# inverted-ai/torchdrivesim

Measured on AMD Instinct MI355X. Metric: agent-steps/sec (whole node) at B=1024xA=64, 256x256 BEV, higher is better.
Workload: dtype f32

## Files before the change

include/tdship.h:

```cpp
#ifndef TDSHIP_H
#define TDSHIP_H

#include <stddef.h>
#include <stdint.h>

#ifdef __cplusplus
extern "C" {
#endif

#define TDS_ABI_VERSION 1

#define TDS_OK 0
#define TDS_EINVAL (-1)
#define TDS_EHIP (-2)
#define TDS_ENOMEM (-3)
#define TDS_ELIMIT (-4)

int tds_version(void);
int tds_last_error(char *buf, size_t n);


int tds_bicycle_step_f32(const float *state, const float *action, const float *lr, float *out, int64_t n,
                         float dt, float max_acc, float max_steer, int left_handed, int no_reversing, void *stream);
int tds_bicycle_step_bwd_f32(const float *state, const float *action, const float *lr, const float *grad_out,
// ... 299 lines not shown
int tds_time_to_collision_f32(const float *boxes, const float *sc, const float *speed, const uint8_t *present, const uint8_t *visible,
                              float *ttc, int32_t *index, int64_t B, int64_t A, int64_t E, int K, float horizon, float margin, void *stream);

int tds_time_to_collision_bwd_f32(const float *boxes, const float *sc, const float *speed, const int32_t *index, const float *g_ttc,
                                  float *g_boxes, float *g_sc, float *g_speed, int64_t B, int64_t A, int64_t E, int K, float margin, void *stream);

#define TDS_RASTER_DBG_NO_STATIC 1
#define TDS_RASTER_DBG_NO_ACTORS 2
#define TDS_RASTER_DBG_NO_STORE 4
#define TDS_RASTER_DBG_NO_EDGES 8
#define TDS_RASTER_DBG_NO_SCAN 16
#define TDS_RASTER_DBG_NO_BINNED 32
#define TDS_RASTER_DBG_NO_BITS 64
#define TDS_RASTER_DBG_STATS 128
#define TDS_RASTER_DBG_NO_EDGE_WALK 256
#define TDS_RASTER_DBG_NO_SETUP 512
#define TDS_RASTER_DBG_NO_PROJECT 1024
#define TDS_RASTER_DBG_MINWG3 2048
#define TDS_RASTER_DBG_XCD_CLOCKS 4096
#define TDS_RASTER_DBG_NO_SPLIT 8192
#define TDS_RASTER_DBG_SPLIT 16384
#define TDS_RASTER_DBG_NO_SHORT_PATH 32768
#define TDS_RASTER_DBG_GRID8 65536
#define TDS_RASTER_DBG_GRID4 131072
#define TDS_RASTER_DBG_WHOLE_4WAVES 262144
#define TDS_RASTER_DBG_NO_8WAVES 524288
#define TDS_RASTER_DBG_WIDEST_STRIPS 1048576
#define TDS_RASTER_DBG_NO_EXTRA_STRIP 2097152
#define TDS_RASTER_DBG_PROLOGUE_TWICE 4194304
#define TDS_RASTER_DBG_DROP_SMALL 8388608
#define TDS_RASTER_DBG_SMALL_FREE_SLOPES 16777216
#define TDS_RASTER_DBG_SMALL_NO_MIDDLE_ROW 33554432
#define TDS_RASTER_DBG_HELPER 67108864
#ifndef TDS_RASTER_SMALL_ROWS
#define TDS_RASTER_SMALL_ROWS 7
#endif

#ifdef TDS_TESTING
int tds_raster_set_strip_width(int tw);
int tds_raster_set_bits_waves(int n);
int tds_raster_set_list_lds(int lds_kb);
int tds_raster_set_list_waves(int waves);
int tds_raster_set_debug(int flags);
int tds_raster_set_helper_min_items(int items_per_workgroup);
int tds_raster_get_helper_stats(unsigned long long *out1);
int tds_raster_get_stats(unsigned long long *out16);
int tds_raster_get_prep_stats(unsigned long long *out2);
int tds_raster_get_small_stats(unsigned long long *out16);
typedef struct {
    int form, tw, strips, twp, nwv, nb, minwg, emit, four_per_cu, persist, tws, lw;
    int64_t lds, lds_s, grid, caps, off_counts, off_lists, off_lists3;
} tds_raster_plan_t;
int tds_raster_plan(int64_t n_img, int res, int out_mode, int n_keys, int keys_listed, int actors, int extra, int want_slices, int64_t workspace_bytes,
                    int cus, int force_tw, int bits_waves, int list_waves, int list_lds_kb, int debug, tds_raster_plan_t *out);
int tds_raster_plan_small_lane(int64_t n_img, int res, int out_mode, int n_keys, int keys_listed, int actors, int extra, int want_slices,
                               int64_t workspace_bytes, int cus, int force_tw, int bits_waves, int list_waves, int list_lds_kb, int debug,
                               int small_faces, int *small_lane);
int tds_testing_set_near_lists(int enabled);
int tds_stop_lines_bwd_set_row_lanes(int lanes);
#endif

#ifdef __cplusplus
}
#endif
#endif
```

torchdrivesim_amd/_native.py:

```python
import contextlib
import ctypes
import enum
import functools
import os
import re
import subprocess

import torch

_HERE = os.path.dirname(os.path.abspath(__file__))
LIB_PATH = os.path.join(_HERE, 'lib', 'libtdship.so')
TESTING_LIB_PATH = os.path.join(_HERE, 'lib', 'libtdship_testing.so')
CSRC = os.path.join(_HERE, 'csrc')

METRIC_IOU, METRIC_DISCS = 0, 1
OUT_F32, OUT_U8 = 0, 1
OUT_MASK_U8, OUT_MASK_BITS = 2, 3
RASTER_NO_TRIM = 1
RASTER_REWRITE_ALL = 2
RASTER_HAS_CAMERA_PREP = 4
RASTER_NO_SMALL_FACES = 8
RASTER_HAS_HELPER_STREAM = 16


class RasterDebug(enum.IntFlag):
    NO_STATIC = 1
    NO_ACTORS = 2
    NO_STORE = 4
    NO_EDGES = 8
    NO_SCAN = 16
    NO_BINNED = 32
    NO_BITS = 64
    STATS = 128
    NO_EDGE_WALK = 256
    NO_SETUP = 512
    NO_PROJECT = 1024
    MINWG3 = 2048
    XCD_CLOCKS = 4096
    NO_SPLIT = 8192
    SPLIT = 16384
    NO_SHORT_PATH = 32768
    GRID8 = 65536
    GRID4 = 131072
    WHOLE_4WAVES = 262144
    NO_8WAVES = 524288
    WIDEST_STRIPS = 1048576
    NO_EXTRA_STRIP = 2097152
    PROLOGUE_TWICE = 4194304
    DROP_SMALL = 8388608
    SMALL_FREE_SLOPES = 16777216
    SMALL_NO_MIDDLE_ROW = 33554432
    HELPER = 67108864

_lib = None


class RasterAux(ctypes.Structure):
    _fields_ = [('index_slices', ctypes.c_void_p), ('index_slices_bytes', ctypes.c_int64), ('keys', ctypes.c_uint32 * 16),
                ('n_keys', ctypes.c_int32), ('index_bits', ctypes.c_int32), ('flags', ctypes.c_int32), ('coverage_maintained', ctypes.c_int32),
                ('coverage', ctypes.c_void_p), ('coverage_bytes', ctypes.c_int64)]


class RasterAuxPrep(RasterAux):
    _fields_ = [('camera_prep', ctypes.c_void_p), ('camera_prep_bytes', ctypes.c_int64)]


class RasterAuxHelper(RasterAuxPrep):
    _fields_ = [('helper_stream', ctypes.c_void_p), ('helper_workgroups', ctypes.c_int64)]


_ABI = '''
tds_version()
tds_last_error(host* buf, size_t n)
tds_bicycle_step_f32(f32* state, f32* action, f32* lr, f32* out, int64 n, float dt, float max_acc, float max_steer, int left_handed, int no_reversing, stream stream)
tds_bicycle_step_bwd_f32(f32* state, f32* action, f32* lr, f32* grad_out, f32* grad_state, f32* grad_action, f32* grad_lr, int64 n, float dt, float max_acc, float max_steer,
    int left_handed, int no_reversing, stream stream)
tds_simple_step_f32(f32* state, f32* action, f32* out, int64 n, float dt, host* norm, int oriented, stream stream)
tds_simple_step_bwd_f32(f32* state, f32* action, f32* grad_out, f32* grad_state, f32* grad_action, int64 n, float dt, host* norm, int oriented, stream stream)
tds_unicycle_step_f32(f32* state, f32* action, f32* out, int64 n, float dt, float max_acc, float max_yaw_rate, stream stream)
tds_unicycle_step_bwd_f32(f32* state, f32* action, f32* grad_out, f32* grad_state, f32* grad_action, int64 n, float dt, float max_acc, float max_yaw_rate, stream stream)
tds_collision_f32(f32* boxes, f32* sc, u8* present, f32* out, i64* overlap, i32* partner, int64 B, int64 A, int64 N, int metric, stream stream)
tds_collision_bwd_f32(f32* boxes, f32* sc, u8* present, f32* grad_out, f32* grad_boxes, f32* grad_sc, int64 B, int64 A, int64 N, int metric, stream stream)
tds_overlap_count_f32(f32* boxes, f32* sc, u8* present, f64* out, int64 B, int64 A, stream stream)
tds_pairwise_overlap_f32(f32* box1, f32* sc1, f32* box2, f32* sc2, f32* out, int64 n, int metric, stream stream)
tds_pairwise_discs_f32(f32* box1, f32* sc1, f32* box2, f32* sc2, f32* out, int64 n, int num_discs, stream stream)
# ... 97 lines not shown
tds_range_scan_multi_f32(handle set, i32* scene_map, f32* boxes, f32* sc, u8* present, f32* ray_sc, f32* agent_range, f32* road_range, i32* hit, int64 B, int64 A, int64 E,
    int R, float max_range, float gap_tolerance, stream stream)
tds_range_scan_bwd_f32(handle map, f32* boxes, f32* sc, u8* present, f32* ray_sc, f32* road_range, f32* g_agent, f32* g_road, f32* g_boxes, f32* g_sc, f32* g_ray_sc,
    i32* choice, f32* road_edge, int64 B, int64 A, int64 E, int R, float max_range, float gap_tolerance, stream stream)
tds_range_scan_bwd_multi_f32(handle set, i32* scene_map, f32* boxes, f32* sc, u8* present, f32* ray_sc, f32* road_range, f32* g_agent, f32* g_road, f32* g_boxes, f32* g_sc,
    f32* g_ray_sc, i32* choice, f32* road_edge, int64 B, int64 A, int64 E, int R, float max_range, float gap_tolerance, stream stream)
tds_neighbors_f32(f32* boxes, f32* sc, f32* speed, u8* present, u8* visible, f32* features, i32* index, int64 B, int64 A, int64 E, int K, float max_distance, stream stream)
tds_neighbors_bwd_f32(f32* boxes, f32* sc, f32* speed, i32* index, f32* g_features, f32* g_boxes, f32* g_sc, f32* g_speed, int64 B, int64 A, int64 E, int K, stream stream)
tds_lights_step(f64* duration, i32* next_phase, i32* n_phases, u8* colour, i32* phase, f64* remaining, i64* state, f32* time_to_change, u8* mask, int64 B, int64 M, int64 P,
    int64 N, host* dt, int advance, stream stream)
tds_lights_reset(i32* n_phases, f64* duration, i32* phase, f64* remaining, u8* mask, i64* scene_ids, int64 B, int64 M, int64 P, uint64 seed, stream stream)
tds_stop_lines_f32(f32* agent_xy, f32* agent_sc, u8* agent_present, f32* lines, f32* line_sc, u8* mask, i64* state, f32* time_to_change, f32* features, i32* index,
    i32* slot_state, int64 B, int64 A, int64 N, int K, float max_distance, int ahead_only, float min_cos, stream stream)
tds_stop_lines_bwd_f32(f32* agent_xy, f32* agent_sc, f32* lines, f32* line_sc, i32* index, f32* g_features, f32* g_xy, f32* g_sc, int64 B, int64 A, int64 N, int K,
    stream stream)
tds_lane_observations_multi(handle set, i32* scene_map, f32* agent_xy, f32* agent_sc, u8* present, f32* features, f32* points, i32* n_valid, i32* index, int64 B, int64 A,
    int K, int P, float spacing, float max_distance, stream stream)
tds_lane_observations_bwd_multi(handle set, i32* scene_map, f32* agent_xy, f32* agent_sc, i32* index, f32* g_features, f32* g_points, f32* g_xy, f32* g_sc, int64 B, int64 A,
    int K, int P, float spacing, stream stream)
tds_time_to_collision_f32(f32* boxes, f32* sc, f32* speed, u8* present, u8* visible, f32* ttc, i32* index, int64 B, int64 A, int64 E, int K, float horizon,
    float margin, stream stream)
tds_time_to_collision_bwd_f32(f32* boxes, f32* sc, f32* speed, i32* index, f32* g_ttc, f32* g_boxes, f32* g_sc, f32* g_speed, int64 B, int64 A, int64 E, int K,
    float margin, stream stream)
'''

_TESTING_ABI = '''
tds_raster_set_strip_width(int tw)
tds_raster_set_bits_waves(int n)
tds_raster_set_list_lds(int lds_kb)
tds_raster_set_list_waves(int waves)
tds_raster_set_debug(int flags)
tds_raster_set_helper_min_items(int items_per_workgroup)
tds_raster_get_helper_stats(host* out1)
tds_raster_get_stats(host* out16)
tds_raster_get_prep_stats(host* out2)
tds_raster_get_small_stats(host* out16)
tds_raster_plan(int64 n_img, int res, int out_mode, int n_keys, int keys_listed, int actors, int extra, int want_slices, int64 workspace_bytes, int cus, int force_tw,
    int bits_waves, int list_waves, int list_lds_kb, int debug, host* out)
tds_raster_plan_small_lane(int64 n_img, int res, int out_mode, int n_keys, int keys_listed, int actors, int extra, int want_slices, int64 workspace_bytes, int cus,
    int force_tw, int bits_waves, int list_waves, int list_lds_kb, int debug, int small_faces, host* small_lane)
tds_testing_set_near_lists(int enabled)
tds_stop_lines_bwd_set_row_lanes(int lanes)
'''

ELEMENTS = {'f32*': torch.float32, 'f64*': torch.float64, 'u8*': torch.uint8, 'i32*': torch.int32, 'i64*': torch.int64, 'void*': None}
SCALARS = {'int': ctypes.c_int, 'int64': ctypes.c_int64, 'uint64': ctypes.c_uint64, 'float': ctypes.c_float, 'size_t': ctypes.c_size_t}


def _parse(abi):
    decls = {name: [tuple(p.split()) for p in params.split(',') if p.strip()] for name, params in re.findall(r'(\w+)\((.*?)\)', abi, flags=re.S)}
    assert all(k in ELEMENTS or k in SCALARS or k in ('host*', 'handle', 'stream') for d in decls.values() for k, _ in d)
    return decls


DECLARATIONS, TESTING_DECLARATIONS = _parse(_ABI), _parse(_TESTING_ABI)
_SIGNATURES = {name: [SCALARS.get(k, ctypes.c_void_p) for k, _ in d] for name, d in DECLARATIONS.items()}
_TESTING_SIGNATURES = {name: [SCALARS.get(k, ctypes.c_void_p) for k, _ in d] for name, d in TESTING_DECLARATIONS.items()}
_RESTYPES = {'tds_buffer_ptr': ctypes.c_void_p, 'tds_torch_alloc': ctypes.c_void_p, 'tds_torch_free': None}


def build(force=False):
    cmd = ['make', '-C', CSRC, '-j', str(min(8, os.cpu_count() or 1))]
    if force:
        cmd.append('-B')
    subprocess.check_call(cmd, stdout=subprocess.DEVNULL)
    return LIB_PATH
# ... 121 lines not shown
```

torchdrivesim_amd/csrc/raster.hip:

```cpp
#include "tds_common.h"
#include "tds_face_rows.h"
#include "tds_raster_plan.h"
#include "tds_short_slope.h"
#include <algorithm>
#include <atomic>
#include <mutex>
#include <type_traits>

using tds::GridEntry;
using tds::MapView;
using namespace tds_raster;

#ifdef TDS_TESTING
#define TDS_DBG(x) (x)
#else
#define TDS_DBG(x) 0
#endif

namespace {

constexpr int RBLOCK = RWAVES * 64;
constexpr int NO_SWITCH = 0x7fffffff;
constexpr int COORD_LIMIT = 16000;

struct SceneArgs {
    MapView map;
    const MapView *views;
    const int32_t *scene_map;
    const float4 *state;
    const float2 *agent_sc;
    const float2 *tmpl;
    const uint32_t *actor_key;
// ... 659 lines not shown
    MapView m = a.map;
    if (a.views != nullptr) m = a.views[a.scene_map[img / a.Nc]];
    int cx0 = 0, cx1 = -1, cy0 = 0, nrows = 0, rtotal = 0;
    if (m.nx > 0 && !(TDS_DBG(c.debug) & TDS_RASTER_DBG_NO_STATIC)) {
        int cy1;
        scan_window(m, c, cam, X0, TWp, cx0, cx1, cy0, cy1);
        nrows = (cx0 <= cx1 && cy0 <= cy1) ? cy1 - cy0 + 1 : 0;
    }
    if (nrows > 0 && nrows <= PREP_ROWS) {
        ScanQuad q;
        scan_quad(q, c, cam, X0, TWp);
        for (int r = 0; r < nrows; ++r) {
            int rw = SCAN_EMPTY_ROW, rfe = 0, re0 = 0, re1 = 0;
            scan_row(q, m, cx0, cx1, cy0, r, rw, rfe, re0, re1);
            rec.rows[r] = make_int4(rw, rtotal, re0 - rtotal, rfe);
            rtotal += re1 - re0;
        }
    }
    float *f = rec.cam;
    f[0] = cam.cx; f[1] = cam.cy; f[2] = cam.s; f[3] = cam.c;
#pragma unroll
    for (int k = 0; k < 4; ++k) { f[4 + k] = cam.px[k]; f[8 + k] = cam.py[k]; }
    rec.cx0 = cx0; rec.cx1 = cx1; rec.cy0 = cy0; rec.nrows = nrows;
    rec.rtotal = rtotal; rec.flags = nrows > PREP_ROWS ? PREP_COMPUTE : 0; rec.pad0 = 0; rec.pad1 = 0;
}

typedef const __attribute__((address_space(4))) int PrepWords;
__device__ __forceinline__ PrepWords *prep_words(const void *tab, int item) {
    return (PrepWords *)((uintptr_t)tab + (uintptr_t)(unsigned)item * sizeof(PrepRecord));
}

template <typename SA, bool POLY = false>
__device__ __forceinline__ void scan_init(ScanState &st, const SA &a, const CommonArgs &c, const Camera &cam, int64_t img, int lane, int wave, int X0,
                                          int TWw, const PrepRecord *rec = nullptr) {
    st.map = a.map;
    if (a.views != nullptr) st.map = a.views[a.scene_map[img / a.Nc]];
    if constexpr (POLY) st.map.cell_start = st.map.qcell_start;
    const MapView &m = st.map;
    st.phase = (a.N > 0 && !(TDS_DBG(c.debug) & TDS_RASTER_DBG_NO_ACTORS)) ? 0 : 2;
    if constexpr (POLY) {
        st.phase = (a.N > 0 && !(c.debug & TDS_RASTER_DBG_NO_ACTORS)) ? 0 : 2;
    }
    if constexpr (has_extras<SA>::value) { if (st.phase == 2 && a.K > 0) st.phase = 3; }
    st.a0 = 0; st.masked_seen = false;
    st.cx0 = 0; st.cx1 = -1; st.cy0 = 0; st.nrows = 0; st.row = 0; st.chunk = __builtin_amdgcn_readfirstlane(wave); st.prev_rw = SCAN_EMPTY_ROW;
    st.rw = SCAN_EMPTY_ROW; st.rex = st.rbase = st.rfe = 0; st.rtotal = 0;
    st.have = false; st.cur_i = -1; st.dyn = nullptr; st.done = 0;
    st.pu0 = st.pu1 = st.pu2 = make_uint4(0, 0, 0, 0);
    if (m.nx > 0 && !(TDS_DBG(c.debug) & TDS_RASTER_DBG_NO_STATIC)) {
        if (rec != nullptr) {
            PrepWords *w = prep_words(rec, 0);
            st.cx0 = w[12]; st.cx1 = w[13]; st.cy0 = w[14]; st.nrows = w[15]; st.rtotal = w[16];
            st.rex = st.rtotal; st.rbase = -st.rtotal;
            if (lane < st.nrows) {
                const int4 v = rec->rows[lane];
                st.rw = v.x; st.rex = v.y; st.rbase = v.z; st.rfe = v.w;
            }
        } else {
            int cy1;
            scan_window(m, c, cam, X0, TWw, st.cx0, st.cx1, st.cy0, cy1);
            st.nrows = (st.cx0 <= st.cx1 && st.cy0 <= cy1) ? __builtin_amdgcn_readfirstlane(cy1 - st.cy0 + 1) : 0;
            if (st.nrows > 0) scan_load_rows(st, m, c, cam, lane, X0, TWw, 0);
        }
    }
}

template <int NW, bool POLY = false>
__device__ __forceinline__ bool scan_fetch(ScanState &st, const MapView &m, const CommonArgs &c, const Camera &cam, int lane, int X0, int TWw) {
    while (st.row < st.nrows) {
        const int nblk = min(64, st.nrows - st.row);
        const int total = st.rtotal;
        if (st.chunk * 64 < total) {
// ... 44 lines not shown
            const int cand = r + step;
            const int ex = __shfl(st.rex, cand & 63);
            if (cand < nblk && ex <= v) r = cand;
        }
    }
    const int i = __shfl(st.rbase, r) + v;
    return v < st.rtotal ? (i | (r << 25)) : -1;
}

__device__ __forceinline__ void scan_candidate(const ScanState &st, const CommonArgs &c, const Camera &cam, int X0, int TWw, int ci, const uint4 &u0,
                                               const uint4 &u1, bool &acc, uint32_t &key, int (&px)[3], int (&py)[3], unsigned &edges) {
    const int i = ci & 0x1ffffff, r = ci >= 0 ? ci >> 25 : 0;
    const int first_end = __shfl(st.rfe, r);
    const int above = __shfl(st.rw, (r + 63) & 63);
    const int pw = r > 0 ? above : st.prev_rw;
    const int plo = pw & 0xffff, phi = pw >> 16;
    const bool top = st.row + r == 0;
    if (ci >= 0) {
        const unsigned own = u1.w;
        const int bx0 = (int)(own & 0x1fffu), bx1 = (int)((own >> 13) & 0x1fffu);
        const bool first_in_row = !(own & (1u << 26)) || (i < first_end);
        const bool none_above = !(own & (1u << 27)) || top || bx1 < plo || bx0 > phi;
        if (first_in_row && none_above && !(TDS_DBG(c.debug) & TDS_RASTER_DBG_NO_PROJECT)) {
            unsigned ins = 0;
            float sxv[3] = {__uint_as_float(u0.x) + (-cam.cx), __uint_as_float(u0.z) + (-cam.cx), __uint_as_float(u1.x) + (-cam.cx)};
            float syv[3] = {__uint_as_float(u0.y) + (-cam.cy), __uint_as_float(u0.w) + (-cam.cy), __uint_as_float(u1.y) + (-cam.cy)};
            key = u1.z;
            acc = trim_project(cam, c.scale, c.res, X0, TWw, sxv, syv, px, py, ins, c.no_trim);
            edges = edge_mask(own >> 29, ins);
        }
    }
}

template <int NW = RWAVES, typename SA = SceneArgsEx>
__device__ __forceinline__ bool scan_step(ScanState &st, const SA &a, const CommonArgs &c, const Camera &cam, int64_t img, int lane,
                                          int wave, int X0, int TWw, bool &acc, uint32_t &key, int (&px)[3], int (&py)[3], unsigned &edges) {
    const MapView &m = st.map;
    unsigned ins = 0;
    edges = 7u;
    const int res = c.res;
    const int64_t b = img / a.Nc;
    acc = false;
    key = 0;
    if (st.phase == 0) {
        const int slot = lane / 3, f = lane - 3 * slot;
        const int ag = st.a0 + slot * NW + wave;
        if (lane < 63 && ag < a.N) {
            const int64_t ia = b * a.N + ag;
            const bool on = a.mask[img * a.N + ag] != 0;
            st.masked_seen = st.masked_seen || !on;
            if (on) {
                const float view_r = 1.05f * 1.41421356f / c.scale;
                const float4 s = a.state[ia];
                const float2 t0 = a.tmpl[ia * 7];
                float reach = view_r + sqrtf(t0.x * t0.x + t0.y * t0.y);
                reach = reach * 1.01f + 0.01f;
                const float ddx = s.x - cam.cx, ddy = s.y - cam.cy;
                if (!(ddx * ddx + ddy * ddy > reach * reach)) {
                    const int64_t ik = a.key_per_cam ? img * a.N + ag : ia;
                    key = a.actor_key[2 * ik + (f == 2 ? 1 : 0)];
                    if (key != 0u) {
                        const float2 sc = a.agent_sc[ia];
                        const int v0 = f == 0 ? 0 : (f == 1 ? 1 : 4), v1 = f == 0 ? 1 : (f == 1 ? 3 : 5), v2 = f == 0 ? 3 : (f == 1 ? 2 : 6);
                        const float2 ta = a.tmpl[ia * 7 + v0], tb = a.tmpl[ia * 7 + v1], tc = a.tmpl[ia * 7 + v2];
                        const float fx[3] = {((sc.y * ta.x + (-sc.x) * ta.y) + s.x) + (-cam.cx), ((sc.y * tb.x + (-sc.x) * tb.y) + s.x) + (-cam.cx),
                                             ((sc.y * tc.x + (-sc.x) * tc.y) + s.x) + (-cam.cx)};
                        const float fy[3] = {((sc.x * ta.x + sc.y * ta.y) + s.y) + (-cam.cy), ((sc.x * tb.x + sc.y * tb.y) + s.y) + (-cam.cy),
                                             ((sc.x * tc.x + sc.y * tc.y) + s.y) + (-cam.cy)};
                        acc = trim_project(cam, c.scale, res, X0, TWw, fx, fy, px, py, ins, c.no_trim);
                        edges = edge_mask(f == 1 ? 2u : 0u, ins);
                    }
                }
            }
        }
        st.a0 += 21 * NW;
        if (st.a0 >= a.N) st.phase = 1;
// ... 461 lines not shown
    if ((c1 & c2) == 0 && (c1 | c2) != 0) {
        int a;
        if (c1 & 12) {
            a = c1 < 8 ? 0 : bottom;
            x1 += clip_quot(a - y1, x2 - x1, y2 - y1);
            y1 = a;
            c1 = (x1 < 0) + (x1 > right) * 2;
        }
        if (c2 & 12) {
            a = c2 < 8 ? 0 : bottom;
            x2 += clip_quot(a - y2, x2 - x1, y2 - y1);
            y2 = a;
            c2 = (x2 < 0) + (x2 > right) * 2;
        }
        if ((c1 & c2) == 0 && (c1 | c2) != 0) {
            if (c1) {
                a = c1 == 1 ? 0 : right;
                y1 += clip_quot(a - x1, y2 - y1, x2 - x1);
                x1 = a;
                c1 = 0;
            }
            if (c2) {
                a = c2 == 1 ? 0 : right;
                y2 += clip_quot(a - x2, y2 - y1, x2 - x1);
                x2 = a;
                c2 = 0;
            }
        }
    }
    return (c1 | c2) == 0;
}

#ifdef TDS_TESTING
__device__ unsigned long long g_stats[19];
__device__ unsigned long long g_small_stats[16];
#define TDS_STAT_LANES(W, I, V) do { if ((W).debug & TDS_RASTER_DBG_STATS) { const unsigned long long v_ = (unsigned long long)(V); if (v_) atomicAdd(&g_stats[I], v_); } } while (0)
#define TDS_STAT(W, I, V) do { if (((W).debug & TDS_RASTER_DBG_STATS) && (W).lane == 0) atomicAdd(&g_stats[I], (unsigned long long)(V)); } while (0)
#else
#define TDS_STAT_LANES(W, I, V) do { } while (0)
#define TDS_STAT(W, I, V) do { } while (0)
#endif
#ifndef TDS_FCHUNK
#define TDS_FCHUNK 4
#endif
#ifndef TDS_VCHUNK
#define TDS_VCHUNK 6
#endif
#ifndef TDS_HCHUNK
#define TDS_HCHUNK 3
#endif
constexpr int CHUNK = TDS_FCHUNK;
constexpr int VCHUNK = TDS_VCHUNK;
constexpr int HCHUNK = TDS_HCHUNK;

constexpr int MERGE_DY_BIAS = 100, MERGE_DY_NOBIAS = 147;

__device__ __forceinline__ unsigned vertex_outcode(int x, int y, int W, int H) {
    return ((unsigned)x >> 31) | (((unsigned)(W - 1 - x) >> 31) << 1) | (((unsigned)y >> 31) << 2) | (((unsigned)(H - 1 - y) >> 31) << 3);
}
__device__ __forceinline__ unsigned edge_class(int ax, int ay, int bx, int by, unsigned oca, unsigned ocb) {
    const bool inside = (oca | ocb) == 0u;
    const int adx = abs(bx - ax), ady = abs(by - ay);
    const bool xmaj = adx >= ady, shortish = ady <= MERGE_DY_BIAS;
    bool merge = inside && shortish;
    const bool longer = inside && !shortish && ady <= MERGE_DY_NOBIAS;
    if (__ballot(longer) != 0) {
        const int fx = __ffs(adx), fy = __ffs(ady);
// ... 765 lines not shown

__device__ __noinline__ void claim_work(uint32_t *queue, int nblk, uint32_t *state, const uint32_t *only, int strips) {
    if (queue == nullptr) {
        int64_t img;
        int strip;
        block_to_image(nblk, strips, img, strip);
        state[0] = state[1] == 0 ? (uint32_t)(img * strips + strip) : 0xffffffffu;
        state[1] = 1;
        return;
    }
    if (only != nullptr) {
        const uint32_t j = atomicAdd(&queue[0], 1u), n = only[0] * (uint32_t)strips;
        state[0] = j < n ? only[1 + j / (uint32_t)strips] * (uint32_t)strips + j % (uint32_t)strips : 0xffffffffu;
        return;
    }
    const int nq = (nblk & 7) == 0 ? 8 : 1, per = nq == 8 ? nblk >> 3 : nblk;
    const int xcd = (int)(__builtin_amdgcn_s_getreg((3 << 11) | 20) & (unsigned)(nq - 1));
    int tried = (int)state[1], item = -1;
    for (; tried < nq; ++tried) {
        const int v = (xcd + tried) & (nq - 1);
        const uint32_t i = atomicAdd(&queue[v], 1u);
        if (i < (uint32_t)per) { item = v * per + (int)i; break; }
    }
    state[1] = (uint32_t)tried;
    state[0] = (uint32_t)item;
}

template <int BWAVES, int NB, typename OutT, typename SA, bool EMIT = false, int MINWG = 3>
__global__ void __launch_bounds__(BWAVES * 64, BWAVES == 4 ? MINWG : 4) raster_scene_bits_kernel(SA a, CommonArgs c, KeyTable kt, int TWp, uint32_t *queue, const uint32_t *only) {
    using E = typename PairTab<NB, OutT>::E;
    constexpr int BBLOCK = BWAVES * 64, P = 1 << (2 * NB);
    constexpr bool PERSIST = BWAVES == 4 && MINWG == 3;
    constexpr int SROWS = PERSIST && !is_mask<OutT>::value ? SMALL_ROWS : 0;
    extern __shared__ __attribute__((aligned(16))) uint32_t smem[];
    const int tid = threadIdx.x, lane = tid & 63, wave = tid >> 6;
    const int res = c.res, H = res, W = res, wpr = TWp >> 5, K = kt.n;
    const int plane_dw = K * H * wpr;
    E *tab = (E *)smem;
    uint32_t *lkeys = smem + pair_tab_dw<NB, OutT>();
    uint32_t *planes = lkeys + BITS_FIXED_DW + BWAVES * BITS_WAVE_LDS_DW;
    if constexpr (PERSIST) {
        if (tid == 0) { lkeys[17] = 0; claim_work(queue, (int)(c.n_img * c.strips), lkeys + 16, only, c.strips); }
    }
#ifdef TDS_TESTING
    if ((c.debug & TDS_RASTER_DBG_XCD_CLOCKS) && tid == 0) atomicMax(&g_stats[8 + (blockIdx.x & 7)], ~(unsigned long long)wall_clock64());
#endif
    if (tid < 16) {
        uint32_t kv = 0xffffffffu;
#pragma unroll
        for (int i = 0; i < 16; ++i) kv = (tid == i) ? kt.key[i] : kv;
        lkeys[tid] = kv;
    }
    __syncthreads();
    if constexpr (!is_mask<OutT>::value) {
        for (int e = tid; e < 3 * P; e += BBLOCK) {
            const int ch = e / P, pr = e - ch * P, ilo = pr & ((1 << NB) - 1), ihi = pr >> NB;
            const uint32_t klo = (ilo >= 1 && ilo <= K) ? lkeys[ilo - 1] : 0u, khi = (ihi >= 1 && ihi <= K) ? lkeys[ihi - 1] : 0u;
            const int sh = 16 - 8 * ch;
            const uint32_t vlo = (klo >> sh) & 255u, vhi = (khi >> sh) & 255u;
            if constexpr (sizeof(OutT) == 4) tab[e] = make_float2((float)vlo, (float)vhi);
            else tab[e] = vlo | (vhi << 8);
        }
    }
    BitCtx w;
    w.planes = planes;
    w.q = lkeys + BITS_FIXED_DW + wave * BITS_WAVE_LDS_DW;
    w.slots = w.q + Q_DW;
    w.eq = w.slots + 64;
    w.lane = lane; w.H = H; w.W = W; w.TWp = TWp; w.wpr = wpr; w.debug = c.debug;
#pragma unroll 1
    for (;;) {
        int64_t img;
        int X0;
        const PrepRecord *rec = nullptr;
        if constexpr (PERSIST) {
            __syncthreads();
            const int item = __builtin_amdgcn_readfirstlane((int)lkeys[16]);
            if (item < 0) break;
            img = item / c.strips;
            X0 = (item - (int)img * c.strips) * TWp;
            if (c.prep != nullptr) {
                rec = (const PrepRecord *)c.prep + item;
                if (prep_words(rec, 0)[17] & PREP_COMPUTE) rec = nullptr;
            }
#ifdef TDS_TESTING
            if ((c.debug & TDS_RASTER_DBG_STATS) && tid == 0) atomicAdd(&g_stats[rec != nullptr ? 16 : 17], 1ull);
            if ((c.debug & TDS_RASTER_DBG_STATS) && (c.debug & TDS_RASTER_DBG_HELPER) && tid == 0) atomicAdd(&g_stats[18], 1ull);
#endif
        } else {
            int strip;
            block_to_image(c.n_img * c.strips, c.strips, img, strip);
            X0 = strip * TWp;
        }
        for (int i = tid * 4; i < plane_dw; i += BBLOCK * 4) *(uint4 *)(planes + i) = make_uint4(0, 0, 0, 0);
        if (tid == 15) lkeys[15] = (uint32_t)BWAVES;
        if constexpr (sizeof(OutT) != 4) __builtin_amdgcn_s_setprio(1);
        w.eq_head = 0; w.eq_count = 0;
        w.slots[lane] = 0;
        w.qlen = 0; w.X0 = X0; w.gen = 0;
        CommonArgs ci = c;
        if constexpr (PERSIST) {
            int sb = __float_as_int(c.scale), rb = c.res;
            asm volatile("" : "+s"(sb), "+s"(rb));
            ci.scale = __int_as_float(sb); ci.res = rb;
        }
        Camera cam;
        if (rec != nullptr) {
            const float4 *f = (const float4 *)rec->cam;
            const float4 f0 = f[0], f1 = f[1], f2 = f[2];
            cam.cx = f0.x; cam.cy = f0.y; cam.s = f0.z; cam.c = f0.w;
            cam.px[0] = f1.x; cam.px[1] = f1.y; cam.px[2] = f1.z; cam.px[3] = f1.w;
            cam.py[0] = f2.x; cam.py[1] = f2.y; cam.py[2] = f2.z; cam.py[3] = f2.w;
        } else {
            float2 xy = c.cam_xy[img], sc = c.cam_sc[img];
            cam.cx = xy.x; cam.cy = xy.y; cam.s = sc.x; cam.c = sc.y;
            polygon_corners(cam, ci.scale, ci.res);
        }
        camera_uniform(cam);
        __syncthreads();
        ScanState st;
        scan_init(st, a, ci, cam, img, lane, wave, X0, TWp, rec);
        st.dyn = lkeys + 15;
#ifdef TDS_TESTING
        if (c.debug & TDS_RASTER_DBG_PROLOGUE_TWICE) {
            CommonArgs c2 = c;
            int sb = __float_as_int(c.scale), rb = c.res;
            float2 xy = c.cam_xy[img], sc = c.cam_sc[img];
            asm volatile("" : "+s"(sb), "+s"(rb), "+v"(xy.x), "+v"(xy.y), "+v"(sc.x), "+v"(sc.y));
            c2.scale = __int_as_float(sb); c2.res = rb;
            Camera cam2;
            cam2.cx = xy.x; cam2.cy = xy.y; cam2.s = sc.x; cam2.c = sc.y;
            make_polygon(cam2, c2.scale, c2.res);
            ScanState st2;
            scan_init(st2, a, c2, cam2, img, lane, wave, X0, TWp);
            float f = 0.0f;
#pragma unroll
            for (int k = 0; k < 4; ++k) f += cam2.px[k] + cam2.py[k];
            const int sink = __float_as_int(f) ^ st2.rw ^ st2.rex ^ st2.rbase ^ st2.rfe ^ st2.rtotal ^ st2.cx0 ^ st2.cx1 ^ st2.cy0 ^ st2.nrows;
            asm volatile("" :: "v"(sink));
        }
#endif
        for (;;) {
            bool acc;
            uint32_t key;
            int px[3] = {0, 0, 0}, py[3] = {0, 0, 0};
            unsigned edges;
            const bool map_phase = st.phase == 2;
            const bool more = scan_step<BWAVES, SA>(st, a, ci, cam, img, lane, wave, X0, TWp, acc, key, px, py, edges);
            drain_bits<true, SROWS>(w, key_plane(lkeys, K, key), acc, edges, px, py, more, map_phase, c.small_lane != 0);
            if (!more) break;
        }
        if constexpr (PERSIST) { if (tid == 0) claim_work(queue, (int)(c.n_img * c.strips), lkeys + 16, only, c.strips); }
        __syncthreads();
        if constexpr (sizeof(OutT) != 4) __builtin_amdgcn_s_setprio(0);
        if (!(TDS_DBG(c.debug) & TDS_RASTER_DBG_NO_STORE)) {
            if constexpr (is_mask<OutT>::value) write_out_masks<BBLOCK, OutT>(planes, c.slices, c.out, img, res, X0, TWp, wpr, tid);
            else {
                constexpr bool TRACK = PERSIST && sizeof(OutT) == 4 && !EMIT;
                write_out_bits<BBLOCK, NB, OutT, EMIT, TRACK>(planes, tab, K, (OutT *)c.out, img, res, X0, TWp, wpr, tid, c.slices);
            }
        }
        if constexpr (!PERSIST) break;
    }
#ifdef TDS_TESTING
    if ((c.debug & TDS_RASTER_DBG_XCD_CLOCKS) && lane == 0) atomicMax(&g_stats[blockIdx.x & 7], (unsigned long long)wall_clock64());
#endif
}

constexpr int SCAN_WAVES = 4;
#ifndef TDS_SMALL_TALL_RES
#define TDS_SMALL_TALL_RES 112
#endif
constexpr int SMALL_TALL_RES = TDS_SMALL_TALL_RES;
#ifndef TDS_SCAN_DEPTH
#define TDS_SCAN_DEPTH 1
#endif
#ifndef TDS_SCAN_OCC
#define TDS_SCAN_OCC 5
#endif
constexpr int SCAN_DEPTH = TDS_SCAN_DEPTH;
constexpr uint32_t LIST_POISON = 0xffffffffu;
// ... 615 lines not shown
    cm.prep = nullptr;
    with_out(out_mode, [&](auto t) { with_tw(tw, [&](auto w) {
        launch(raster_mesh_kernel<w, decltype(t)>, n_img * cm.strips, RBLOCK, lds_bytes(w, res), (hipStream_t)stream, a, cm);
    }); });
    TDS_LAUNCH_CHECK("raster_mesh_kernel");
    return TDS_OK;
}

#ifdef TDS_TESTING
TDS_EXPORT int tds_raster_get_stats(unsigned long long *out16) {
    TDS_CHECK_ARG(out16, "tds_raster_get_stats: null output");
    unsigned long long zero[16] = {0};
    if (hipMemcpyFromSymbol(out16, HIP_SYMBOL(g_stats), sizeof(zero)) != hipSuccess) { tds::set_error("tds_raster_get_stats: copy failed"); return TDS_EHIP; }
    if (hipMemcpyToSymbol(HIP_SYMBOL(g_stats), zero, sizeof(zero)) != hipSuccess) { tds::set_error("tds_raster_get_stats: reset failed"); return TDS_EHIP; }
    return TDS_OK;
}

TDS_EXPORT int tds_raster_get_prep_stats(unsigned long long *out2) {
    TDS_CHECK_ARG(out2, "tds_raster_get_prep_stats: null output");
    unsigned long long zero[2] = {0, 0};
    if (hipMemcpyFromSymbol(out2, HIP_SYMBOL(g_stats), sizeof(zero), 16 * sizeof(unsigned long long)) != hipSuccess) { tds::set_error("tds_raster_get_prep_stats: copy failed"); return TDS_EHIP; }
    if (hipMemcpyToSymbol(HIP_SYMBOL(g_stats), zero, sizeof(zero), 16 * sizeof(unsigned long long)) != hipSuccess) { tds::set_error("tds_raster_get_prep_stats: reset failed"); return TDS_EHIP; }
    return TDS_OK;
}

TDS_EXPORT int tds_raster_get_helper_stats(unsigned long long *out1) {
    TDS_CHECK_ARG(out1, "tds_raster_get_helper_stats: null output");
    unsigned long long zero[1] = {0};
    if (hipMemcpyFromSymbol(out1, HIP_SYMBOL(g_stats), sizeof(zero), 18 * sizeof(unsigned long long)) != hipSuccess) { tds::set_error("tds_raster_get_helper_stats: copy failed"); return TDS_EHIP; }
    if (hipMemcpyToSymbol(HIP_SYMBOL(g_stats), zero, sizeof(zero), 18 * sizeof(unsigned long long)) != hipSuccess) { tds::set_error("tds_raster_get_helper_stats: reset failed"); return TDS_EHIP; }
    return TDS_OK;
}

TDS_EXPORT int tds_raster_get_small_stats(unsigned long long *out16) {
    TDS_CHECK_ARG(out16, "tds_raster_get_small_stats: null output");
    unsigned long long zero[16] = {0};
    if (hipMemcpyFromSymbol(out16, HIP_SYMBOL(g_small_stats), sizeof(zero)) != hipSuccess) { tds::set_error("tds_raster_get_small_stats: copy failed"); return TDS_EHIP; }
    if (hipMemcpyToSymbol(HIP_SYMBOL(g_small_stats), zero, sizeof(zero)) != hipSuccess) { tds::set_error("tds_raster_get_small_stats: reset failed"); return TDS_EHIP; }
    return TDS_OK;
}
#endif
#endif
```

Measured before the change: 12.84 million.

## Rasterize actors in a single wave per strip with ballot-compacted visible agents

In the persistent raster kernel, only one wave per work item (chosen by item index modulo four) runs the actor phase. That wave culls all 64 agents of a round with a distance test, compacts the visible ones through a ballot and an LDS slot table, and emits three faces per agent for up to 21 agents per step. The other waves skip straight to the map phase. This avoids each wave scanning many off-screen agents and lets the waves overlap actor and map work. The cost is load imbalance across waves and an extra wave sync per step.

```diff
diff --git a/include/tdship.h b/include/tdship.h
--- a/include/tdship.h
+++ b/include/tdship.h
@@ -355,6 +355,7 @@
 #define TDS_RASTER_DBG_SMALL_FREE_SLOPES 16777216
 #define TDS_RASTER_DBG_SMALL_NO_MIDDLE_ROW 33554432
 #define TDS_RASTER_DBG_HELPER 67108864
+#define TDS_RASTER_DBG_NO_ACTOR_WAVE 134217728
 #ifndef TDS_RASTER_SMALL_ROWS
 #define TDS_RASTER_SMALL_ROWS 7
 #endif
@@ -367,6 +368,7 @@
 int tds_raster_set_debug(int flags);
 int tds_raster_set_helper_min_items(int items_per_workgroup);
 int tds_raster_get_helper_stats(unsigned long long *out1);
+int tds_raster_get_actor_wave_stats(unsigned long long *out1);
 int tds_raster_get_stats(unsigned long long *out16);
 int tds_raster_get_prep_stats(unsigned long long *out2);
 int tds_raster_get_small_stats(unsigned long long *out16);
diff --git a/torchdrivesim_amd/_native.py b/torchdrivesim_amd/_native.py
--- a/torchdrivesim_amd/_native.py
+++ b/torchdrivesim_amd/_native.py
@@ -51,6 +51,7 @@
     SMALL_FREE_SLOPES = 16777216
     SMALL_NO_MIDDLE_ROW = 33554432
     HELPER = 67108864
+    NO_ACTOR_WAVE = 134217728
 
 _lib = None
 
@@ -214,6 +215,7 @@
 tds_raster_set_debug(int flags)
 tds_raster_set_helper_min_items(int items_per_workgroup)
 tds_raster_get_helper_stats(host* out1)
+tds_raster_get_actor_wave_stats(host* out1)
 tds_raster_get_stats(host* out16)
 tds_raster_get_prep_stats(host* out2)
 tds_raster_get_small_stats(host* out16)
diff --git a/torchdrivesim_amd/csrc/raster.hip b/torchdrivesim_amd/csrc/raster.hip
--- a/torchdrivesim_amd/csrc/raster.hip
+++ b/torchdrivesim_amd/csrc/raster.hip
@@ -1,3 +1,4 @@
+#include "tds_actor_lanes.h"
 #include "tds_common.h"
 #include "tds_face_rows.h"
 #include "tds_raster_plan.h"
@@ -723,12 +724,12 @@
 
 template <typename SA, bool POLY = false>
 __device__ __forceinline__ void scan_init(ScanState &st, const SA &a, const CommonArgs &c, const Camera &cam, int64_t img, int lane, int wave, int X0,
-                                          int TWw, const PrepRecord *rec = nullptr) {
+                                          int TWw, const PrepRecord *rec = nullptr, bool actors = true) {
     st.map = a.map;
     if (a.views != nullptr) st.map = a.views[a.scene_map[img / a.Nc]];
     if constexpr (POLY) st.map.cell_start = st.map.qcell_start;
     const MapView &m = st.map;
-    st.phase = (a.N > 0 && !(TDS_DBG(c.debug) & TDS_RASTER_DBG_NO_ACTORS)) ? 0 : 2;
+    st.phase = (a.N > 0 && actors && !(TDS_DBG(c.debug) & TDS_RASTER_DBG_NO_ACTORS)) ? 0 : 2;
     if constexpr (POLY) {
         st.phase = (a.N > 0 && !(c.debug & TDS_RASTER_DBG_NO_ACTORS)) ? 0 : 2;
     }
@@ -839,9 +840,10 @@
     }
 }
 
-template <int NW = RWAVES, typename SA = SceneArgsEx>
+template <int NW = RWAVES, typename SA = SceneArgsEx, bool ACTW = false>
 __device__ __forceinline__ bool scan_step(ScanState &st, const SA &a, const CommonArgs &c, const Camera &cam, int64_t img, int lane,
-                                          int wave, int X0, int TWw, bool &acc, uint32_t &key, int (&px)[3], int (&py)[3], unsigned &edges) {
+                                          int wave, int X0, int TWw, bool &acc, uint32_t &key, int (&px)[3], int (&py)[3], unsigned &edges,
+                                          uint32_t *slots = nullptr) {
     const MapView &m = st.map;
     unsigned ins = 0;
     edges = 7u;
@@ -849,6 +851,50 @@
     const int64_t b = img / a.Nc;
     acc = false;
     key = 0;
+    if constexpr (ACTW) if (st.phase == 0 && !(TDS_DBG(c.debug) & TDS_RASTER_DBG_NO_ACTOR_WAVE)) {
+        const int step = st.a0 & (TDS_ACTOR_ROUND - 1), cand = st.a0 - step + lane;
+        bool off = false, seen = false;
+        if (cand < a.N) {
+            const int64_t ia = b * a.N + cand;
+            off = a.mask[img * a.N + cand] == 0;
+            if (!off) {
+                const float view_r = 1.05f * 1.41421356f / c.scale;
+                const float4 s = a.state[ia];
+                const float2 t0 = a.tmpl[ia * 7];
+                float reach = view_r + sqrtf(t0.x * t0.x + t0.y * t0.y);
+                reach = reach * 1.01f + 0.01f;
+                const float ddx = s.x - cam.cx, ddy = s.y - cam.cy;
+                seen = !(ddx * ddx + ddy * ddy > reach * reach);
+            }
+        }
+        st.masked_seen = st.masked_seen || __ballot(off) != 0;
+        const uint64_t vis = __ballot(seen);
+        const int drop = actor_drop_position(vis, lane, step);
+        if (drop >= 0) slots[drop] = (uint32_t)lane;
+        wave_sync();
+        const int pos = actor_lane_position(vis, lane, step), f = actor_lane_face(lane);
+        if (pos >= 0) {
+            const int ag = st.a0 - step + (int)slots[pos];
+            const int64_t ia = b * a.N + ag;
+            const int64_t ik = a.key_per_cam ? img * a.N + ag : ia;
+            key = a.actor_key[2 * ik + (f == 2 ? 1 : 0)];
+            if (key != 0u) {
+                const float4 s = a.state[ia];
+                const float2 sc = a.agent_sc[ia];
+                const int v0 = f == 0 ? 0 : (f == 1 ? 1 : 4), v1 = f == 0 ? 1 : (f == 1 ? 3 : 5), v2 = f == 0 ? 3 : (f == 1 ? 2 : 6);
+                const float2 ta = a.tmpl[ia * 7 + v0], tb = a.tmpl[ia * 7 + v1], tc = a.tmpl[ia * 7 + v2];
+                const float fx[3] = {((sc.y * ta.x + (-sc.x) * ta.y) + s.x) + (-cam.cx), ((sc.y * tb.x + (-sc.x) * tb.y) + s.x) + (-cam.cx),
+                                     ((sc.y * tc.x + (-sc.x) * tc.y) + s.x) + (-cam.cx)};
+                const float fy[3] = {((sc.x * ta.x + sc.y * ta.y) + s.y) + (-cam.cy), ((sc.x * tb.x + sc.y * tb.y) + s.y) + (-cam.cy),
+                                     ((sc.x * tc.x + sc.y * tc.y) + s.y) + (-cam.cy)};
+                acc = trim_project(cam, c.scale, res, X0, TWw, fx, fy, px, py, ins, c.no_trim);
+                edges = edge_mask(f == 1 ? 2u : 0u, ins);
+            }
+        }
+        st.a0 = actor_more_steps(vis, step) ? st.a0 + 1 : st.a0 - step + TDS_ACTOR_ROUND;
+        if (st.a0 >= a.N) st.phase = 1;
+        return true;
+    }
     if (st.phase == 0) {
         const int slot = lane / 3, f = lane - 3 * slot;
         const int ag = st.a0 + slot * NW + wave;
@@ -1376,7 +1422,7 @@
 }
 
 #ifdef TDS_TESTING
-__device__ unsigned long long g_stats[19];
+__device__ unsigned long long g_stats[20];
 __device__ unsigned long long g_small_stats[16];
 #define TDS_STAT_LANES(W, I, V) do { if ((W).debug & TDS_RASTER_DBG_STATS) { const unsigned long long v_ = (unsigned long long)(V); if (v_) atomicAdd(&g_stats[I], v_); } } while (0)
 #define TDS_STAT(W, I, V) do { if (((W).debug & TDS_RASTER_DBG_STATS) && (W).lane == 0) atomicAdd(&g_stats[I], (unsigned long long)(V)); } while (0)
@@ -2208,6 +2254,7 @@
     constexpr int BBLOCK = BWAVES * 64, P = 1 << (2 * NB);
     constexpr bool PERSIST = BWAVES == 4 && MINWG == 3;
     constexpr int SROWS = PERSIST && !is_mask<OutT>::value ? SMALL_ROWS : 0;
+    constexpr bool ACTW = PERSIST;
     extern __shared__ __attribute__((aligned(16))) uint32_t smem[];
     const int tid = threadIdx.x, lane = tid & 63, wave = tid >> 6;
     const int res = c.res, H = res, W = res, wpr = TWp >> 5, K = kt.n;
@@ -2249,10 +2296,12 @@
         int64_t img;
         int X0;
         const PrepRecord *rec = nullptr;
+        int item_no = 0;
         if constexpr (PERSIST) {
             __syncthreads();
             const int item = __builtin_amdgcn_readfirstlane((int)lkeys[16]);
             if (item < 0) break;
+            item_no = item;
             img = item / c.strips;
             X0 = (item - (int)img * c.strips) * TWp;
             if (c.prep != nullptr) {
@@ -2294,9 +2343,16 @@
         }
         camera_uniform(cam);
         __syncthreads();
+        bool actors = true;
+        if constexpr (ACTW) actors = (TDS_DBG(c.debug) & TDS_RASTER_DBG_NO_ACTOR_WAVE) != 0 || __builtin_amdgcn_readfirstlane(wave) == (item_no & 3);
         ScanState st;
-        scan_init(st, a, ci, cam, img, lane, wave, X0, TWp, rec);
+        scan_init(st, a, ci, cam, img, lane, wave, X0, TWp, rec, actors);
         st.dyn = lkeys + 15;
+#ifdef TDS_TESTING
+        if constexpr (ACTW) {
+            if ((c.debug & TDS_RASTER_DBG_STATS) && !(c.debug & TDS_RASTER_DBG_NO_ACTOR_WAVE) && st.phase == 0 && lane == 0) atomicAdd(&g_stats[19], 1ull);
+        }
+#endif
 #ifdef TDS_TESTING
         if (c.debug & TDS_RASTER_DBG_PROLOGUE_TWICE) {
             CommonArgs c2 = c;
@@ -2322,7 +2378,7 @@
             int px[3] = {0, 0, 0}, py[3] = {0, 0, 0};
             unsigned edges;
             const bool map_phase = st.phase == 2;
-            const bool more = scan_step<BWAVES, SA>(st, a, ci, cam, img, lane, wave, X0, TWp, acc, key, px, py, edges);
+            const bool more = scan_step<BWAVES, SA, ACTW>(st, a, ci, cam, img, lane, wave, X0, TWp, acc, key, px, py, edges, w.slots);
             drain_bits<true, SROWS>(w, key_plane(lkeys, K, key), acc, edges, px, py, more, map_phase, c.small_lane != 0);
             if (!more) break;
         }
@@ -3004,6 +3060,14 @@
     return TDS_OK;
 }
 
+TDS_EXPORT int tds_raster_get_actor_wave_stats(unsigned long long *out1) {
+    TDS_CHECK_ARG(out1, "tds_raster_get_actor_wave_stats: null output");
+    unsigned long long zero[1] = {0};
+    if (hipMemcpyFromSymbol(out1, HIP_SYMBOL(g_stats), sizeof(zero), 19 * sizeof(unsigned long long)) != hipSuccess) { tds::set_error("tds_raster_get_actor_wave_stats: copy failed"); return TDS_EHIP; }
+    if (hipMemcpyToSymbol(HIP_SYMBOL(g_stats), zero, sizeof(zero), 19 * sizeof(unsigned long long)) != hipSuccess) { tds::set_error("tds_raster_get_actor_wave_stats: reset failed"); return TDS_EHIP; }
+    return TDS_OK;
+}
+
 TDS_EXPORT int tds_raster_get_small_stats(unsigned long long *out16) {
     TDS_CHECK_ARG(out16, "tds_raster_get_small_stats: null output");
     unsigned long long zero[16] = {0};
diff --git a/torchdrivesim_amd/csrc/tds_actor_lanes.h b/torchdrivesim_amd/csrc/tds_actor_lanes.h
--- /dev/null
+++ b/torchdrivesim_amd/csrc/tds_actor_lanes.h
@@ -0,0 +1,40 @@
+#pragma once
+#include <stdint.h>
+
+#ifdef __HIPCC__
+#define TDS_AL_HD __host__ __device__
+#else
+#define TDS_AL_HD
+#endif
+
+#define TDS_ACTOR_FACES 3
+#define TDS_ACTOR_STEP_AGENTS 21
+#define TDS_ACTOR_ROUND 64
+
+TDS_AL_HD __inline__ __attribute__((always_inline)) int actor_popcount(uint64_t v) {
+    return __builtin_popcountll(v);
+}
+TDS_AL_HD __inline__ __attribute__((always_inline)) int actor_rank(uint64_t vis, int j) {
+#ifdef __HIP_DEVICE_COMPILE__
+    (void)j;
+    return (int)__builtin_amdgcn_mbcnt_hi((unsigned)(vis >> 32), __builtin_amdgcn_mbcnt_lo((unsigned)vis, 0u));
+#else
+    return actor_popcount(vis & (((uint64_t)1 << j) - 1u));
+#endif
+}
+TDS_AL_HD __inline__ __attribute__((always_inline)) int actor_round_agents(int N, int r) {
+    const int left = N - TDS_ACTOR_ROUND * r;
+    return left < 0 ? 0 : (left > TDS_ACTOR_ROUND ? TDS_ACTOR_ROUND : left);
+}
+TDS_AL_HD __inline__ __attribute__((always_inline)) int actor_drop_position(uint64_t vis, int j, int step) {
+    const int rel = actor_rank(vis, j) - TDS_ACTOR_STEP_AGENTS * step;
+    return ((vis >> j) & 1u) && rel >= 0 && rel < TDS_ACTOR_STEP_AGENTS ? rel : -1;
+}
+TDS_AL_HD __inline__ __attribute__((always_inline)) int actor_lane_position(uint64_t vis, int lane, int step) {
+    const int slot = lane / TDS_ACTOR_FACES;
+    return lane < TDS_ACTOR_FACES * TDS_ACTOR_STEP_AGENTS && TDS_ACTOR_STEP_AGENTS * step + slot < actor_popcount(vis) ? slot : -1;
+}
+TDS_AL_HD __inline__ __attribute__((always_inline)) int actor_lane_face(int lane) { return lane - TDS_ACTOR_FACES * (lane / TDS_ACTOR_FACES); }
+TDS_AL_HD __inline__ __attribute__((always_inline)) bool actor_more_steps(uint64_t vis, int step) {
+    return actor_popcount(vis) > TDS_ACTOR_STEP_AGENTS * (step + 1);
+}
```

Result: faster. 13.27 million, median of 6 (+3.3%).
